# mpotse/ParMmg

Hardware: AMD Instinct MI355X
Metric: new-mesh points located+interpolated/sec (Mpts/s) and HBM GB/s, 1/2/4/8 GPU (higher is better)
Workload: dtype f64

## Files before the change

parmmg_amd/csrc/pmmg_hip.hip:

```cpp
#include <hip/hip_ext.h>
#include <hip/hip_runtime.h>
#ifdef PMMG_HIP_MEASURE
#include <rocprim/device/device_radix_sort.hpp>
#endif

#include <math.h>
#include <stdarg.h>
#include <stdint.h>
#include <stdio.h>
#include <stdlib.h>
#include <string.h>

#include <algorithm>
#include <chrono>
#include <condition_variable>
#include <functional>
#include <mutex>
#include <string>
#include <thread>
#include <type_traits>
#include <vector>

#include "pmmg_device.hpp"
#include "pmmg_prep.hpp"
// ... 93 lines not shown
  st->sorted = sorted;
  st->bin_bits = bits;
}
#endif

}


struct DevBuf {
  void *p = nullptr;
  size_t cap = 0;
};

enum {
  EV_START, EV_FRAME, EV_PREP, EV_ORDER, EV_VOL0, EV_WALK, EV_VOL, EV_JOIN, EV_END, EV_BDY0, EV_BDY1, EV_RESET,
  EV_SB0, EV_ORDER2, EV_SRFSEED, EV_FILL, EV_BDYFB, EV_QUANT, EV_COUNT
};

struct pmmg_hip_ctx {
  int device = 0;
  int options = 0;
  hipStream_t stream = nullptr;
  hipStream_t stream2 = nullptr;
  hipStream_t stream3 = nullptr;
  hipStream_t stream_f = nullptr;
  hipStream_t stream2_hi = nullptr;
  bool srf_prio = false;
  char err[512] = {0};
  Bg bg{};
  int met_size = 0;
  int nfield = 0;
  std::vector<int> fsize;
  std::vector<const double *> fin;
  const double *met = nullptr;
  const double *rec = nullptr;
  int rstride = 0;
  DevBuf o_xyz, o_tetv, o_adja, o_triv, o_adjt, o_met, o_rec;
  std::vector<DevBuf> o_f;
  DevBuf frame, stats, grid, sgrid, order_v, order_b, cont, xq;
  DevBuf cohd;
  DevBuf axh;
  DevBuf bkeys, bkeys2, bvals, bvals2;
  DevBuf rs_hist, rs_csum;
  DevBuf brk_k, brk_k2, brk_v, brk_v2, brk_vinv, brk_tinv, brk_xq, brk_xyz, brk_sol, brk_rec, brk_tmp;
  int brick = 0;
  int set_order = 0;
  int no_fb = 0;
  int stream3_mode = 1;
  int srf_solo = -1;
  void *grid_clean_p = nullptr, *sgrid_clean_p = nullptr;
  long long grid_clean_n = 0, sgrid_clean_n = 0;
  DevBuf qs;
  DevBuf cls_cnt;
  DevBuf oflag;
  DevBuf qmin;
  DevBuf fb_vol, fb_bdy, best, nac, cres, bbest, bnac, bcres;
  DevBuf fbp_vol, fbp_bdy;
  DevBuf fbg_vol_c, fbg_vol_u, fbg_vol_i, fbg_bdy_c, fbg_bdy_u, fbg_bdy_i;
  DevBuf h_xyz, h_cls, h_met, h_elem, h_hit;
  std::vector<DevBuf> h_f;
  hipEvent_t ev[EV_COUNT] = {};
  bool pending = false;
  void *stage[2] = {nullptr, nullptr};
  void *stage_dev[2] = {nullptr, nullptr};
  hipEvent_t stage_ev[2] = {};
  int stage_i = 0;
  struct Pool *pool = nullptr;
  DevBuf o_tet4;
  SnapCache snap_cache;
  hipStream_t cstream = nullptr;
  std::thread snap;
  int snap_ok = 1;
  int verbose = 0;
  int tpc = 8;
  int seed_lanes = 4;
  int seed_v0 = 0;
  int pack_passes = 0;
  int bbox_stride = 64;
  int hist_stride = 256;
  int bdy_bpx = 512;
  int bdy_wave = 0;
  int ev_vol0 = EV_VOL0, ev_vol = EV_VOL;
  int quant_side = 0;
  int fuse_cont = 1;
  int host_order = 1;
  int *flag_host = nullptr;
  int *flag_host_dev = nullptr;
  int bdy_dyn = 0;
  int srf_g = 0;
  int srf_mult = 8;
  int bin_bits = kBinBitsCoherent;
  int bin_qs = 0;
  int maxstep = 1024;
  int fanmax = kFanMax;
  int pad = 0;
  int xcd_run = 64;
  struct Kept {
    DevBuf xyz, met;
    std::vector<DevBuf> f;
    int np = 0, met_size = 0;
    std::vector<int> fsize;
    bool valid = false;
  };
  std::vector<Kept> kept;
  int last_host_np = 0, last_host_met = 0;
  std::vector<int> last_host_fsize;
  int carry_slot = -1, carry_np = 0;
  bool carry_bg = false;
  std::vector<int> carry_src;
  DevBuf carry_dsrc, carry_need, carry_ids, carry_cnt, carry_rows, carry_bc;
  int64_t bytes_up = 0;
  std::vector<pmmg_hip_ctx *> lanes;
  bool borrowed_streams = false;
  ncclComm_t comm = nullptr;
  bool comm_owned = false;
  int comm_rank = 0, comm_size = 0;
  DevBuf ag_send, ag_recv, ag_off, ag_chk;
  int group_lanes = 3;
  struct Pool *lane_pool = nullptr;
  int lane_streams = 1;
  int bdy_first = 0;
  int bdy_after = 0;
  int vol_wait_seed = 0;
  int lane0 = 1;
  int vol_split = 0;
  DevBuf locv, locp;
  static constexpr int kMaxVolChunks = 16;
  int vol_chunks = 4;
  hipStream_t stream_i = nullptr;
  hipEvent_t ev_chunk[2][kMaxVolChunks] = {};
  hipEvent_t ev_interp = nullptr;
  int ixcd_run = -1;
  int null_sync = 0;
  int eager_lanes = 0;
  int wave_time = 0;
  DevBuf wt;
  size_t wt_n = 0;
  int filter_steps = 64;
};

static void set_err(pmmg_hip_ctx *c, const char *fmt, ...) {
  if (!c) return;
  va_list ap;
  va_start(ap, fmt);
  vsnprintf(c->err, sizeof(c->err), fmt, ap);
  va_end(ap);
  fprintf(stderr, "[parmmg_hip] %s\n", c->err);
}

#define HIPCK(ctx, expr)                                                                             \
  do {                                                                                               \
    hipError_t e_ = (expr);                                                                          \
    if (e_ != hipSuccess) {                                                                          \
      set_err((ctx), "%s failed: %s (%s:%d)", #expr, hipGetErrorString(e_), __FILE__, __LINE__);   \
      return 0;                                                                                      \
    }                                                                                                \
  } while (0)

static hipError_t ctx_d2h(pmmg_hip_ctx *c, void *dst, const void *src, size_t n) {
  if (c->null_sync) return hipMemcpy(dst, src, n, hipMemcpyDeviceToHost);
  hipError_t e = hipMemcpyAsync(dst, src, n, hipMemcpyDeviceToHost, c->stream);
  return e != hipSuccess ? e : hipStreamSynchronize(c->stream);
}

static int ensure(pmmg_hip_ctx *c, DevBuf &b, size_t bytes) {
  if (bytes == 0) bytes = 16;
// ... 238 lines not shown
}
constexpr long long kRefillCells = 1LL << 20;

static int env_int(const char *name, int def) {
  const char *e = getenv(name);
  if (e && atoi(e) > 0) return atoi(e);
  return def;
}
static int env_int_any(const char *name, int def) {
  const char *e = getenv(name);
  if (!e || !*e) return def;
  char *end = nullptr;
  const long v = strtol(e, &end, 10);
  return (end && *end == 0) ? (int)v : def;
}

extern "C" {

int pmmg_hip_abi_version(void) { return PMMG_HIP_ABI_VERSION; }
int64_t pmmg_hip_stats_size(void) { return (int64_t)sizeof(pmmg_hip_stats); }

int pmmg_hip_device_count(void) {
  int n = 0;
  if (hipGetDeviceCount(&n) != hipSuccess) return 0;
  return n;
}

static pmmg_hip_ctx *create_ctx(int device, int options, bool srf_prio, pmmg_hip_ctx *share = nullptr) {
  int n = pmmg_hip_device_count();
  if (n <= 0 || device < 0 || device >= n) {
    fprintf(stderr, "[parmmg_hip] no HIP device %d (visible: %d)\n", device, n);
    return nullptr;
  }
  pmmg_hip_ctx *c = new pmmg_hip_ctx();
  c->device = device;
  c->options = options;
#ifdef PMMG_HIP_MEASURE
  if (const char *e = getenv("PMMG_HIP_SRFPRIO"))
    if (*e == '1') c->srf_prio = srf_prio;
#else
  (void)srf_prio;
#endif
  if (share) {
    c->stream = share->stream;
    c->stream2 = share->stream2;
    c->borrowed_streams = true;
  }
  if (hipSetDevice(device) != hipSuccess ||
      (!share && (hipStreamCreateWithFlags(&c->stream, hipStreamNonBlocking) != hipSuccess ||
                  hipStreamCreateWithFlags(&c->stream2, hipStreamNonBlocking) != hipSuccess))) {
    fprintf(stderr, "[parmmg_hip] cannot initialise device %d\n", device);
    delete c;
    return nullptr;
  }
  {
    int evf = 0;
#ifdef PMMG_HIP_MEASURE
    evf = env_int("PMMG_HIP_EVFLAGS", 0);
#endif
    const unsigned fl = evf == 1 ? hipEventDisableSystemFence : (evf == 2 ? hipEventReleaseToDevice : 0u);
    for (int i = 0; i < EV_COUNT; i++)
      (void)hipEventCreateWithFlags(&c->ev[i], (i == EV_FRAME || i == EV_END) ? hipEventDefault : fl);
  }
  c->tpc = std::min(4096, env_int("PMMG_HIP_TPC", c->tpc));
  c->srf_mult = std::min(4096, env_int("PMMG_HIP_SRFMULT", c->srf_mult));
  c->bin_bits = std::min(7, env_int("PMMG_HIP_BINBITS", c->bin_bits));
  c->verbose = env_int("PMMG_HIP_VERBOSE", 0);
  c->maxstep = env_int("PMMG_HIP_MAXSTEP", c->maxstep);
  c->group_lanes = std::min(16, env_int("PMMG_HIP_GROUP_LANES", c->group_lanes));
  c->fanmax = env_int("PMMG_HIP_FANMAX", c->fanmax);
  c->srf_g = std::min(1024, env_int("PMMG_HIP_SRFG", 0));
  c->pack_passes = std::max(0, std::min(2, env_int("PMMG_HIP_PACKPASS", c->pack_passes)));
  if (const char *e = getenv("PMMG_HIP_VOLSPLIT"))
    if (*e == '0' || *e == '1') c->vol_split = *e - '0';
  c->vol_chunks = std::max(1, std::min((int)pmmg_hip_ctx::kMaxVolChunks, env_int("PMMG_HIP_VOLCHUNKS", c->vol_chunks)));
  c->bg.fanmax = c->fanmax;
  c->filter_steps = c->filter_steps < c->maxstep ? c->filter_steps : c->maxstep;
  if (const char *e = getenv("PMMG_HIP_FILTER_STEPS"))
    if (*e && atoi(e) >= 0) c->filter_steps = atoi(e);
#ifdef PMMG_HIP_MEASURE
  c->seed_lanes = std::min(4, env_int("PMMG_HIP_SEEDLANES", c->seed_lanes));
  c->seed_v0 = (env_int("PMMG_HIP_SEEDV0", 0) == 1 ? 1 : 0) | (env_int("PMMG_HIP_SEEDNOATOM", 0) == 1 ? 2 : 0);
  c->bbox_stride = env_int("PMMG_HIP_BBOX", c->bbox_stride);
  c->hist_stride = env_int("PMMG_HIP_HIST", c->hist_stride);
  c->bdy_dyn = (env_int("PMMG_HIP_BDYDYN", 2) == 1 ? 1 : 0) | (env_int("PMMG_HIP_BDYNOINTERP", 0) == 1 ? 2 : 0);
  c->bdy_bpx = env_int("PMMG_HIP_BDYBPX", c->bdy_bpx);
  c->bdy_wave = env_int("PMMG_HIP_BDYWAVE", c->bdy_wave);
  c->host_order = env_int_any("PMMG_HIP_HOSTORDER", c->host_order);
  c->fuse_cont = env_int_any("PMMG_HIP_FUSECONT", c->fuse_cont);
  c->quant_side = env_int("PMMG_HIP_QUANTSIDE", c->quant_side);
  c->bin_qs = env_int("PMMG_HIP_BINQS", 2) == 1;
  c->brick = env_int("PMMG_HIP_BRICK", 0);
  c->srf_solo = env_int_any("PMMG_HIP_SRFSOLO", -1);
  c->set_order = env_int("PMMG_HIP_SETORDER", 0);
  if (const char *e = getenv("PMMG_HIP_XCDRUN"))
    if (*e && atoi(e) >= 0) c->xcd_run = atoi(e);
  c->pad = env_int("PMMG_HIP_PAD", 0);
  c->ixcd_run = env_int_any("PMMG_HIP_IXCDRUN", -1);
  c->null_sync = env_int("PMMG_HIP_NULLSYNC", 0);
  c->eager_lanes = env_int("PMMG_HIP_EAGERLANES", 0);
  c->wave_time = env_int("PMMG_HIP_WAVETIME", 0);
  c->lane_streams = std::max(1, std::min(3, env_int("PMMG_HIP_LANE_STREAMS", c->lane_streams)));
  c->lane0 = env_int_any("PMMG_HIP_LANE0", 1) ? 1 : 0;
  c->bdy_first = env_int("PMMG_HIP_BDYFIRST", 0);
  c->bdy_after = env_int("PMMG_HIP_BDYAFTER", 0);
  c->vol_wait_seed = env_int("PMMG_HIP_VOLWAIT", 0);
  c->no_fb = env_int("PMMG_HIP_NOFB", 0);
  c->stream3_mode = env_int_any("PMMG_HIP_STREAM3", c->stream3_mode);
  if (c->stream3_mode == 2 && hipStreamCreateWithFlags(&c->stream3, hipStreamNonBlocking) != hipSuccess)
    c->stream3 = nullptr;
#endif
  return c;
}

static pmmg_hip_ctx *group_lane(pmmg_hip_ctx *c, int j);

pmmg_hip_ctx *pmmg_hip_create(int device, int options) {
  pmmg_hip_ctx *c = create_ctx(device, options, true);
  if (c && c->eager_lanes)
    for (int j = 0; j < c->group_lanes; j++) (void)group_lane(c, j);
  return c;
}

void pmmg_hip_destroy(pmmg_hip_ctx *c) {
  if (!c) return;
  delete c->lane_pool;
  for (pmmg_hip_ctx *l : c->lanes) pmmg_hip_destroy(l);
  (void)hipSetDevice(c->device);
  (void)snap_join(c);
  (void)hipStreamSynchronize(c->stream);
  (void)hipStreamSynchronize(c->stream2);
  if (c->stream2_hi) (void)hipStreamSynchronize(c->stream2_hi);
  if (c->stream3) (void)hipStreamSynchronize(c->stream3);
  if (c->stream_f) (void)hipStreamSynchronize(c->stream_f);
  if (c->cstream) (void)hipStreamSynchronize(c->cstream);
  if (c->stream_i) {
    (void)hipStreamSynchronize(c->stream_i);
    (void)hipStreamDestroy(c->stream_i);
  }
  for (auto &row : c->ev_chunk)
    for (hipEvent_t &e : row)
      if (e) (void)hipEventDestroy(e);
  if (c->ev_interp) (void)hipEventDestroy(c->ev_interp);
  DevBuf *bufs[] = {&c->o_xyz, &c->o_tetv, &c->o_adja, &c->o_triv, &c->o_adjt, &c->o_met, &c->o_rec, &c->frame,
                    &c->stats, &c->grid, &c->sgrid, &c->order_v, &c->cohd,
                    &c->order_b, &c->cont, &c->xq, &c->qs, &c->axh, &c->bkeys, &c->bkeys2, &c->bvals, &c->bvals2, &c->rs_hist, &c->rs_csum, &c->oflag, &c->cls_cnt, &c->qmin, &c->fb_vol, &c->fb_bdy,
                    &c->best, &c->nac, &c->cres, &c->bbest, &c->bnac, &c->bcres, &c->fbp_vol, &c->fbp_bdy, &c->fbg_vol_c,
                    &c->fbg_vol_u, &c->fbg_vol_i, &c->fbg_bdy_c, &c->fbg_bdy_u, &c->fbg_bdy_i, &c->h_xyz,
                    &c->h_cls, &c->h_met, &c->h_elem, &c->h_hit, &c->brk_k, &c->brk_k2, &c->brk_v, &c->brk_v2,
                    &c->brk_vinv, &c->brk_tinv, &c->brk_xq, &c->brk_xyz, &c->brk_sol, &c->brk_rec, &c->brk_tmp,
                    &c->locv, &c->locp, &c->wt};
  for (DevBuf *b : bufs) release(*b);
  for (auto &b : c->o_f) release(b);
  for (auto &b : c->h_f) release(b);
  for (int i = 0; i < EV_COUNT; i++)
    if (c->ev[i]) (void)hipEventDestroy(c->ev[i]);
  for (int b = 0; b < 2; b++) {
    if (c->stage[b]) (void)hipHostFree(c->stage[b]);
    if (c->stage_ev[b]) (void)hipEventDestroy(c->stage_ev[b]);
  }
  delete c->pool;
  release(c->o_tet4);
  pmmg_snap_cache_free(&c->snap_cache);
  for (auto &k : c->kept) {
    release(k.xyz);
    release(k.met);
// ... 578 lines not shown
    }
    S.s[S.n++] = Slot{c->fin[j], rec_out ? nullptr : fields_out[j], c->fsize[j], c->fsize[j], c->fsize[j]};
  }
  if (c->rec) {
    S.rec = c->rec;
    int off = 0;
    for (int j = 0; j < S.n; j++) {
      S.s[j].in = c->rec + off;
      S.s[j].istride = c->rstride;
      if (rec_out) {
        S.s[j].out = rec_out + off;
        S.s[j].ostride = c->rstride;
      }
      off += S.s[j].code;
    }
    S.rec_out = rec_out;
  }
  const VolPick vpick = pick_layout(S, c->pack_passes);
  if (!vpick.fn) {
    set_err(c, "locate_interp: no packed-record kernel for this slot layout");
    return 0;
  }
  const bool vsplit = S.n > 0 && vpick.ifn && (c->vol_split < 0 ? np_new >= kSmallGroup : c->vol_split == 1);
  LocBuf lb{nullptr, nullptr, nullptr};
  if (vsplit) {
    if (!ensure(c, c->locv, 16 * (size_t)np_new) || !ensure(c, c->locp, 32 * (size_t)np_new)) return 0;
    lb = LocBuf{(nti4 *)c->locv.p, (ntd2 *)c->locp.p, (ntd2 *)c->locp.p + np_new};
    if (!c->stream_i) HIPCK(c, hipStreamCreateWithFlags(&c->stream_i, hipStreamNonBlocking));
    for (auto &row : c->ev_chunk)
      for (hipEvent_t &e : row)
        if (!e) HIPCK(c, hipEventCreateWithFlags(&e, hipEventDisableTiming));
    if (!c->ev_interp) HIPCK(c, hipEventCreateWithFlags(&c->ev_interp, hipEventDisableTiming));
  }
  const VolFn vol_fn = vsplit ? kVolWalk : vpick.fn;
  const int g = grid_dim(bg.ne, c->tpc, 1024);
  const int gs = bg.nt <= 0 ? 1 : (c->srf_g > 0 ? c->srf_g : grid_dim((long long)bg.nt * c->srf_mult, 2, 1024));
  const int gb = 1 << kBinBitsAxis;
  const size_t nq = (size_t)np_new;
  const long long ng = (long long)g * g * g, nsg = bg.nt > 0 ? (long long)gs * gs * gs : 0;
  const long long ncls = (long long)(nq / kScanChunk + 1);
  if (!ensure(c, c->frame, sizeof(Frame)) || !ensure(c, c->stats, sizeof(DevStats) + kStatParts * sizeof(StatPart)) ||
      !ensure(c, c->grid, 8 * (size_t)ng) || !ensure(c, c->sgrid, 8 * (size_t)nsg) || !ensure(c, c->order_v, 4 * nq) ||
      !ensure(c, c->order_b, 4 * nq) || !ensure(c, c->cont, sizeof(ContEntry) * nq) ||
      !ensure(c, c->bkeys, 4 * nq) || !ensure(c, c->bkeys2, 4 * nq) || !ensure(c, c->bvals, 4 * nq) ||
      !ensure(c, c->qs, 24 * nq) || !ensure(c, c->cls_cnt, 4 * (size_t)ncls) || 
      !ensure(c, c->fb_vol, 4 * nq) || !ensure(c, c->fb_bdy, 4 * nq) || !ensure(c, c->best, 4 * nq) ||
      !ensure(c, c->nac, 4 * nq) || !ensure(c, c->cres, 4 * nq) || !ensure(c, c->bbest, 4 * nq) ||
      !ensure(c, c->bnac, 4 * nq) || !ensure(c, c->bcres, 4 * nq) ||
      !ensure(c, c->fbp_vol, sizeof(FbPart) * (size_t)kFbPartCap) ||
      !ensure(c, c->fbp_bdy, sizeof(FbPart) * 256 * (size_t)kFbGridBdy) ||
      !ensure(c, c->fbg_vol_c, 4 * (size_t)(kFbCells + 1)) || !ensure(c, c->fbg_vol_u, 4 * (size_t)kFbCells) ||
      !ensure(c, c->fbg_vol_i, 4 * nq) || !ensure(c, c->fbg_bdy_c, 4 * (size_t)(kFbCells + 1)) ||
      !ensure(c, c->fbg_bdy_u, 4 * (size_t)kFbCells) || !ensure(c, c->fbg_bdy_i, 4 * nq))
    return 0;
  if (!ensure(c, c->xq, sizeof(int) * kXqStride * (size_t)bg.np) || !ensure(c, c->oflag, 2 * sizeof(int)) ||
      !ensure(c, c->cohd, sizeof(double) * kCohSamples) ||
      !ensure(c, c->axh, sizeof(int) * 3 * kMapBins * (size_t)kHistBlocks))
    return 0;
  bg.xq = (const int *)c->xq.p;
  Frame *fr = (Frame *)c->frame.p;
  DevStats *st = (DevStats *)c->stats.p;
  unsigned long long *grid = (unsigned long long *)c->grid.p;
  unsigned long long *sgrid = (unsigned long long *)c->sgrid.p;
  int *order_v = (int *)c->order_v.p, *order_b = (int *)c->order_b.p;
  int force = (c->options & PMMG_HIP_OPT_SORT) ? 1 : (c->options & PMMG_HIP_OPT_NOSORT) ? 0 : -1;
  if (force < 0 && np_new < kSmallGroup) force = 0;
  const bool host_order = force < 0 && c->host_order;
  if (host_order && !c->flag_host) {
    void *p = nullptr;
    HIPCK(c, hipHostMalloc(&p, 64, hipHostMallocCoherent | hipHostMallocMapped));
    c->flag_host = (int *)p;
    void *d = nullptr;
    HIPCK(c, hipHostGetDevicePointer(&d, p, 0));
    c->flag_host_dev = (int *)d;
  }
  if (host_order) c->flag_host[0] = -1;

  const long long ng_clr = (c->grid.p == c->grid_clean_p && ng <= c->grid_clean_n) ? 0 : ng;
  const long long nsg_clr = (c->sgrid.p == c->sgrid_clean_p && nsg <= c->sgrid_clean_n) ? 0 : nsg;
  c->grid_clean_n = c->sgrid_clean_n = 0;
  hipExtLaunchKernelGGL(k_reset, dim3(blocks_for(ng_clr > nsg_clr ? ng_clr : nsg_clr, 2048)), dim3(kBlock), 0, s,
                        c->ev[EV_START], force >= 0 ? c->ev[EV_RESET] : nullptr, 0, fr, st, grid, ng_clr, sgrid,
                        nsg_clr, (int *)c->oflag.p, force, c->bin_bits);
  hipExtLaunchKernelGGL(k_bbox, dim3(std::max(force < 0 ? kCohBlocks : 1, blocks_for(bg.np / c->bbox_stride + 1, 256))),
                        dim3(kBlock), 0, s, nullptr, c->ev[EV_FRAME], 0, (const double *)bg.xyz, bg.np, fr,
                        c->bbox_stride, g, gs, gb, xyz_new, np_new, force < 0 ? (int *)c->oflag.p : nullptr,
                        (double *)c->cohd.p, host_order ? c->flag_host_dev : nullptr);
  const bool quant_side = c->quant_side && np_new >= kSmallGroup;
  if (quant_side) {
    if (!c->stream_f) HIPCK(c, hipStreamCreateWithFlags(&c->stream_f, hipStreamNonBlocking));
    HIPCK(c, hipStreamWaitEvent(c->stream_f, c->ev[EV_FRAME], 0));
    hipLaunchKernelGGL(k_quantize, dim3(blocks_for(3LL * bg.np, 8192)), dim3(kBlock), 0, c->stream_f, bg.xyz,
                       (long long)bg.np, (const Frame *)fr, (int *)c->xq.p, c->hist_stride, (int *)nullptr);
    HIPCK(c, hipEventRecord(c->ev[EV_QUANT], c->stream_f));
    hipLaunchKernelGGL(k_axis_hist, dim3(kHistBlocks), dim3(kBlock), 0, s, bg.xyz, (long long)bg.np,
                       (const Frame *)fr, c->hist_stride, (int *)c->axh.p);
  } else {
    hipLaunchKernelGGL(k_quantize, dim3(std::max(kHistBlocks, blocks_for(3LL * bg.np, 8192))), dim3(kBlock), 0, s,
                       bg.xyz, (long long)bg.np, (const Frame *)fr, (int *)c->xq.p, c->hist_stride, (int *)c->axh.p);
  }
  hipLaunchKernelGGL(k_axis_map, dim3(3), dim3(kBlock), 0, s, (const int *)c->axh.p, fr, g);
  HIPCK(c, hipGetLastError());

  HIPCK(c, hipStreamWaitEvent(sb, c->ev[force < 0 ? EV_FRAME : EV_RESET], 0));
  if (force == 1 || bg.nt <= 0) HIPCK(c, hipEventRecord(c->ev[EV_SB0], sb));
  hipStream_t sc = sb;
  if (force != 0) {
    if (c->stream3_mode == 1 && !c->stream3 &&
        hipStreamCreateWithFlags(&c->stream3, hipStreamNonBlocking) != hipSuccess)
      c->stream3 = nullptr;
    if (c->stream3) sc = c->stream3;
    HIPCK(c, hipStreamWaitEvent(sc, c->ev[EV_FRAME], 0));
  }
  bool split = force < 0 && sc != sb && np_new < (1 << 23);
  HIPCK(c, hipGetLastError());

  {
    const long long nsamp = ng < bg.ne ? ng : bg.ne;
    hipExtLaunchKernelGGL(k_seed_vol, dim3((blocks_for((nsamp + kSeedBatch - 1) / kSeedBatch, 8192) + 7) & ~7),
                          dim3(kBlock), 0, s, nullptr, quant_side ? nullptr : c->ev[EV_PREP], 0, bg, fr, grid, g,
                          nsamp, c->seed_lanes, c->seed_v0, quant_side ? bg.xyz : (const double *)nullptr);
    if (quant_side) {
      HIPCK(c, hipStreamWaitEvent(s, c->ev[EV_QUANT], 0));
      HIPCK(c, hipEventRecord(c->ev[EV_PREP], s));
    }
  }
  HIPCK(c, hipGetLastError());

  const int *flag = (const int *)c->oflag.p;
#ifdef PMMG_HIP_MEASURE
  if (c->set_order) hipLaunchKernelGGL(k_set_order, dim3(1), dim3(1), 0, s, st, force > 0 ? 1 : 0, c->bin_bits);
#endif
  auto launch_cls = [&](bool order_end) -> bool {
    if (force == 1 || bg.nt <= 0) return false;
    int *bc = (int *)c->cls_cnt.p;
    hipExtLaunchKernelGGL(k_cls_count, dim3((unsigned)ncls), dim3(kBlock), 0, sb, c->ev[EV_SB0], nullptr, 0,
                          pclass, (long long)np_new, (int)PMMG_PT_BDY, bc, flag, 0);
    hipLaunchKernelGGL(k_scan_top, dim3(1), dim3(kBlock), 0, sb, bc, (int)ncls, &st->nbdy, flag, 0);
    hipExtLaunchKernelGGL(k_cls_scatter, dim3((unsigned)ncls), dim3(kBlock), 0, sb, nullptr,
                          order_end ? c->ev[EV_ORDER] : nullptr, 0, pclass, (long long)np_new, (int)PMMG_PT_BDY,
                          (const int *)bc, order_b, flag, 0);
    return order_end;
  };
  auto launch_morton = [&]() -> int {
    if (force == 0 || np_new <= 0) return 1;
    const int ntile = (int)((np_new + kRsTile - 1) / kRsTile);
    const long long nh = 256LL * ntile;
    const int nch = (int)((nh + kScanChunk - 1) / kScanChunk);
    if (!ensure(c, c->bvals2, 4 * nq) || !ensure(c, c->rs_hist, 4 * (size_t)nh) || !ensure(c, c->rs_csum, 4 * (size_t)nch))
      return 0;
    unsigned *k0 = (unsigned *)c->bkeys.p, *k1 = (unsigned *)c->bkeys2.p;
    int *v0 = (int *)c->bvals.p, *v1 = (int *)c->bvals2.p, *hist = (int *)c->rs_hist.p, *csum = (int *)c->rs_csum.p;
    const int tgrid = std::min(ntile, kRsGrid);
    hipLaunchKernelGGL(k_bin_keys, dim3(tgrid), dim3(kBlock), 0, sc, xyz_new, pclass, np_new, (const Frame *)fr, flag,
                       k0, v0, st, kRsTile, ntile, hist);
    for (int pass = 0; pass < 3; pass++) {
      const unsigned *kin = pass == 1 ? k1 : k0;
      const int *vin = pass == 1 ? v1 : v0;
      unsigned *kout = pass == 1 ? k0 : k1;
      int *vout = pass == 1 ? v0 : (pass == 0 ? v1 : order_v);
      if (pass > 0)
        hipLaunchKernelGGL(k_rs_hist, dim3(tgrid), dim3(kBlock), 0, sc, kin, np_new, 8 * pass, ntile, hist, flag, 1);
      hipLaunchKernelGGL(k_rs_scan_local, dim3(nch), dim3(kBlock), 0, sc, hist, (int)nh, csum, flag, 1);
      hipLaunchKernelGGL(k_scan_top, dim3(1), dim3(kBlock), 0, sc, csum, nch, (int *)nullptr, flag, 1);
      hipLaunchKernelGGL(k_rs_scan_add, dim3(nch), dim3(kBlock), 0, sc, hist, (int)nh, (const int *)csum, flag, 1);
      hipLaunchKernelGGL(k_rs_scatter, dim3(tgrid), dim3(kBlock), 0, sc, kin, vin, np_new, 8 * pass, ntile,
                         (const int *)hist, kout, vout, flag, 1);
// ... 958 lines not shown
```

parmmg_amd/csrc/pmmg_prep.hpp:

```cpp
#pragma once

#include "pmmg_device.hpp"

namespace pmmg {

struct DevStats {
  int nvol, nbdy;
  int nfb_vol, nfb_bdy;
  int ncont;
  int sorted;
  int bin_bits;
  int pad;
  int bdy_next[8];
  int nac_vol, nac_bdy;
  double fbg_lo[2][3], fbg_inv[2][3];
  int fbg_n[2];
  unsigned walk_done;
  unsigned bdy_done;
  unsigned fb_done[4];
};

struct FbInit {
  int *best;
  __device__ __forceinline__ void at(int slot) const { best[slot] = INT_MAX; }
};

constexpr int kStatParts = 256;
constexpr int kCntVolQueries = 12;
constexpr int kCntWaveIters = 13;
constexpr int kCntExact = 14;
constexpr int kCntNoSeed = 15;
constexpr int kCntStuck = 16;
constexpr int kCntLimit = 17;
constexpr int kCntFanScan = 18;
constexpr int kNumCnt = 20;
struct StatPart {
  unsigned long long cnt[kNumCnt];
  unsigned long long steps;
  unsigned long long stepmax;
};
__device__ __forceinline__ StatPart *stat_part(DevStats *st) {
  return reinterpret_cast<StatPart *>(st + 1) + (blockIdx.x & (kStatParts - 1));
}

struct BlockStats {
  unsigned int cnt[kNumCnt];
  unsigned long long steps;
  unsigned int stepmax;
};

__device__ __forceinline__ void bstats_init(BlockStats *b) {
  if (threadIdx.x < kNumCnt) b->cnt[threadIdx.x] = 0;
  if (threadIdx.x == 0) {
    b->steps = 0;
    b->stepmax = 0;
  }
}

__device__ __forceinline__ void bstats_flush(BlockStats *b, DevStats *st) {
  StatPart *pt = stat_part(st);
  if (threadIdx.x < kNumCnt && b->cnt[threadIdx.x]) atomicAdd(&pt->cnt[threadIdx.x], (unsigned long long)b->cnt[threadIdx.x]);
  if (threadIdx.x == 0) {
    if (b->steps) atomicAdd(&pt->steps, b->steps);
    if (b->stepmax) atomicMax(&pt->stepmax, (unsigned long long)b->stepmax);
  }
}

__device__ __forceinline__ void wave_stats(BlockStats *bs, bool active, int hit, int steps) {
  unsigned int s = active ? (unsigned)steps : 0u, mx = s;
  for (int off = 32; off > 0; off >>= 1) {
    s += __shfl_down(s, off);
    unsigned o = __shfl_down(mx, off);
    mx = o > mx ? o : mx;
  }
  if (__lane_id() == 0) {
    if (s) atomicAdd(&bs->steps, (unsigned long long)s);
    if (mx) {
      atomicMax(&bs->stepmax, mx);
      atomicAdd(&bs->cnt[kCntWaveIters], mx);
    }
  }
  int h = active ? hit : 0;
  unsigned long long any = __ballot(h > 0);
  while (any) {
    int first = __shfl(h, __ffsll((long long)any) - 1);
    unsigned long long same = __ballot(h == first);
    if (__lane_id() == 0) atomicAdd(&bs->cnt[first], (unsigned)__popcll(same));
    any &= ~same;
  }
}

__device__ __forceinline__ void wave_count(BlockStats *bs, int slot, bool pred) {
  const unsigned long long m = __ballot(pred);
  if (__lane_id() == 0 && m) atomicAdd(&bs->cnt[slot], (unsigned)__popcll(m));
}

constexpr int kMapBins = 2048;
constexpr int kMapRatio = 4;
constexpr int kHistBlocks = 32;

constexpr int kSeedAnyParts = 64;
struct Frame {
  unsigned long long key_lo[3], key_hi[3];
  double lo[3], ext[3];
  double inv_vol[3], inv_srf[3], inv_bin[3];
  double qc[3], qs;
  int adaptive;
  int seed_any[kSeedAnyParts];
  unsigned bbox_done;
  float map[3][kMapBins + 1];
};

__device__ __forceinline__ double seed_pos(const Frame *fr, int d, double x, int g) {
  const double u = (x - fr->lo[d]) * fr->inv_vol[d];
  if (!((fr->adaptive >> d) & 1)) return u;
  double b = u * ((double)kMapBins / (double)g);
  b = b > 0.0 ? (b < (double)kMapBins ? b : (double)kMapBins - 1e-9) : 0.0;
  const int i = (int)b;
  const double m0 = fr->map[d][i], m1 = fr->map[d][i + 1];
  return (m0 + (b - (double)i) * (m1 - m0)) * (double)g;
}
__device__ __forceinline__ int seed_cell(double t, int g) {
  const int c = t > 0.0 ? (int)t : 0;
  return c < g ? c : g - 1;
}

constexpr double kQuantHalf = 536870912.0;
__device__ __forceinline__ int quant(double x, const Frame *fr, int d) {
  double t = (x - fr->qc[d]) * fr->qs;
  t = t > 2.0 * kQuantHalf ? 2.0 * kQuantHalf : (t < -2.0 * kQuantHalf ? -2.0 * kQuantHalf : t);
  return __double2int_rn(t);
}

__device__ __forceinline__ void axis_hist_block(int (*h)[kMapBins], const double *xyz, long long np, const Frame *fr,
                                                int stride, int *H) {
  for (int j = threadIdx.x; j < 3 * kMapBins; j += kBlock) (&h[0][0])[j] = 0;
  __syncthreads();
  const long long ns = (np + stride - 1) / stride;
  for (long long j = blockIdx.x * (long long)blockDim.x + threadIdx.x; j < ns; j += (long long)kHistBlocks * blockDim.x) {
    unsigned long long z = (unsigned long long)j * 0x9E3779B97F4A7C15ULL + 0x5EED2025ULL;
    z = (z ^ (z >> 30)) * 0xBF58476D1CE4E5B9ULL;
    z = (z ^ (z >> 27)) * 0x94D049BB133111EBULL;
    z ^= z >> 31;
    const long long i = (long long)(z % (unsigned long long)np);
#pragma unroll
    for (int d = 0; d < 3; d++) {
      const double e = fr->ext[d];
      const double b = e > 0.0 ? (xyz[3 * i + d] - fr->lo[d]) * ((double)kMapBins / e) : 0.0;
      if (b >= 0.0 && b < (double)kMapBins) atomicAdd(&h[d][(int)b], 1);
    }
  }
  __syncthreads();
  for (int j = threadIdx.x; j < 3 * kMapBins; j += kBlock) H[(size_t)blockIdx.x * 3 * kMapBins + j] = (&h[0][0])[j];
}

constexpr int kQuantU = 4;
__global__ __launch_bounds__(kBlock) void k_axis_hist(const double *xyz, long long np, const Frame *fr, int hstride,
                                                      int *H) {
  __shared__ int h[3][kMapBins];
  axis_hist_block(h, xyz, np, fr, hstride, H);
}

__global__ __launch_bounds__(kBlock) void k_quantize(const double *xyz, long long np, const Frame *fr, int *xq,
                                                     int hstride, int *H) {
  __shared__ int h[3][kMapBins];
  if (H && blockIdx.x < kHistBlocks) axis_hist_block(h, xyz, np, fr, hstride, H);
  const long long nth = (long long)gridDim.x * blockDim.x;
  if (kXqStride == 3 && ((uintptr_t)xyz & 15) == 0 && ((uintptr_t)xq & 7) == 0) {
    const double qs = fr->qs, qc0 = fr->qc[0], qc1 = fr->qc[1], qc2 = fr->qc[2];
    const double lim = 2.0 * kQuantHalf;
    auto q = [&](double x, unsigned d) {
      double t = (x - (d == 0 ? qc0 : (d == 1 ? qc1 : qc2))) * qs;
      t = t > lim ? lim : (t < -lim ? -lim : t);
      return __double2int_rn(t);
    };
    const long long n = 3 * np, npair = n / 2;
    const ntd2 *src = reinterpret_cast<const ntd2 *>(xyz);
    nti2 *dst = reinterpret_cast<nti2 *>(xq);
    for (long long p0 = blockIdx.x * (long long)blockDim.x * kQuantU + threadIdx.x; p0 < npair;
         p0 += nth * kQuantU) {
      ntd2 v[kQuantU];
#pragma unroll
      for (int u = 0; u < kQuantU; u++) {
        const long long p = p0 + (long long)u * blockDim.x;
        if (p < npair) v[u] = __builtin_nontemporal_load(src + p);
      }
#pragma unroll
      for (int u = 0; u < kQuantU; u++) {
        const long long p = p0 + (long long)u * blockDim.x;
        if (p < npair) {
          const unsigned d0 = (unsigned)((2 * p) % 3);
          const unsigned d1 = d0 == 2u ? 0u : d0 + 1u;
          const nti2 w = {q(v[u].x, d0), q(v[u].y, d1)};
          __builtin_nontemporal_store(w, dst + p);
        }
      }
    }
    if (blockIdx.x == 0 && threadIdx.x == 0 && (n & 1))
      xq[n - 1] = q(xyz[n - 1], (unsigned)((n - 1) % 3));
    return;
  }
  for (long long j = blockIdx.x * (long long)blockDim.x + threadIdx.x; j < 3 * np; j += nth)
    xq[kXqStride * (j / 3) + j % 3] = quant(__builtin_nontemporal_load(xyz + j), fr, (int)(j % 3));
}

__global__ __launch_bounds__(kBlock) void k_reset(Frame *fr, DevStats *st, unsigned long long *grid, long long ng,
                                                  unsigned long long *sgrid, long long nsg, int *flag, int force,
                                                  int force_bits) {
  const long long tid = blockIdx.x * (long long)blockDim.x + threadIdx.x, nth = (long long)gridDim.x * blockDim.x;
  if (tid < kSeedAnyParts) fr->seed_any[tid] = INT_MAX;
  if (tid == 0) {
    for (int d = 0; d < 3; d++) {
      fr->key_lo[d] = ~0ULL;
      fr->key_hi[d] = 0ULL;
    }
    fr->adaptive = 0;
    fr->bbox_done = 0u;
    if (force >= 0) {
      flag[0] = force;
      flag[1] = force_bits;
    }
    unsigned int *w = reinterpret_cast<unsigned int *>(st);
    for (size_t j = 0; j < sizeof(DevStats) / 4; j++) w[j] = 0u;
  }
  {
    unsigned long long *pw = reinterpret_cast<unsigned long long *>(st + 1);
    for (long long j = tid; j < (long long)(kStatParts * sizeof(StatPart) / 8); j += nth) pw[j] = 0ULL;
  }
  for (long long j = tid; j < ng; j += nth) grid[j] = ~0ULL;
  for (long long j = tid; j < nsg; j += nth) sgrid[j] = ~0ULL;
}

__device__ void frame_final(Frame *fr, int g, int gs, int gb);

constexpr int kCohBlocks = 8, kCohSamples = 4096;
__device__ void coherence_final(const Frame *fr, const double *cohd, int nq, int *flag, int *flag_host);
__device__ __forceinline__ double coh_sample(const double *xyz, int np, int smp) {
  unsigned long long z = (unsigned long long)smp * 0x9E3779B97F4A7C15ULL + 0x5EED2025ULL;
  z = (z ^ (z >> 30)) * 0xBF58476D1CE4E5B9ULL;
  z = (z ^ (z >> 27)) * 0x94D049BB133111EBULL;
  z ^= z >> 31;
  const long long i = (long long)(z % (unsigned long long)(np - 1));
  double d2 = 0.0;
  for (int d = 0; d < 3; d++) {
    const double t = xyz[3 * (size_t)(i + 1) + d] - xyz[3 * (size_t)i + d];
    d2 += t * t;
  }
  return sqrt(d2);
}
__global__ __launch_bounds__(kBlock) void k_bbox(const double *xyz, int np, Frame *fr, int stride, int g, int gs,
                                                 int gb, const double *qxyz, int nq, int *flag, double *cohd,
                                                 int *flag_host) {
  __shared__ unsigned long long slo[3][kBlock / 64], shi[3][kBlock / 64];
  unsigned long long lo[3] = {~0ULL, ~0ULL, ~0ULL}, hi[3] = {0ULL, 0ULL, 0ULL};
  const long long ns = ((long long)np + stride - 1) / stride + 2;
  if (flag && blockIdx.x < kCohBlocks && nq >= 2) {
#pragma unroll
    for (int s = 0; s < kCohSamples / (kCohBlocks * kBlock); s++) {
      const int smp = (blockIdx.x * (kCohSamples / (kCohBlocks * kBlock)) + s) * kBlock + threadIdx.x;
      cohd[smp] = coh_sample(qxyz, nq, smp);
    }
  }
  constexpr int kBboxBatch = 4;
  const long long gs_ = (long long)gridDim.x * blockDim.x;
  for (long long j0 = blockIdx.x * blockDim.x + threadIdx.x; j0 < ns; j0 += kBboxBatch * gs_) {
    double r[kBboxBatch][3];
    bool ok[kBboxBatch];
#pragma unroll
    for (int b = 0; b < kBboxBatch; b++) {
      const long long j = j0 + b * gs_;
      ok[b] = j < ns;
      unsigned long long z = (unsigned long long)j * 0x9E3779B97F4A7C15ULL + 0xB0B0B0B0ULL;
      z = (z ^ (z >> 30)) * 0xBF58476D1CE4E5B9ULL;
      z = (z ^ (z >> 27)) * 0x94D049BB133111EBULL;
      z ^= z >> 31;
      const long long i = !ok[b] || j == 0 ? 0 : (j == 1 ? np - 1 : (long long)(z % (unsigned long long)np));
#pragma unroll
      for (int d = 0; d < 3; d++) r[b][d] = xyz[3 * i + d];
    }
#pragma unroll
    for (int b = 0; b < kBboxBatch; b++)
#pragma unroll
      for (int d = 0; d < 3; d++) {
        const unsigned long long k = dkey(r[b][d]);
        lo[d] = ok[b] && k < lo[d] ? k : lo[d];
        hi[d] = ok[b] && k > hi[d] ? k : hi[d];
      }
  }
#pragma unroll
  for (int d = 0; d < 3; d++) {
    for (int off = 32; off > 0; off >>= 1) {
      unsigned long long a = __shfl_down(lo[d], off), b = __shfl_down(hi[d], off);
      lo[d] = a < lo[d] ? a : lo[d];
      hi[d] = b > hi[d] ? b : hi[d];
    }
  }
  int w = threadIdx.x >> 6, lane = threadIdx.x & 63;
  if (lane == 0)
    for (int d = 0; d < 3; d++) {
      slo[d][w] = lo[d];
      shi[d][w] = hi[d];
    }
  __syncthreads();
  if (threadIdx.x < 3) {
    int d = threadIdx.x;
    unsigned long long a = ~0ULL, b = 0ULL;
    for (int j = 0; j < kBlock / 64; j++) {
      a = slo[d][j] < a ? slo[d][j] : a;
      b = shi[d][j] > b ? shi[d][j] : b;
    }
    atomicMin(&fr->key_lo[d], a);
    atomicMax(&fr->key_hi[d], b);
  }
  __threadfence();
  __syncthreads();
  __shared__ bool last;
  if (threadIdx.x == 0) last = atomicAdd(&fr->bbox_done, 1u) == gridDim.x - 1;
  __syncthreads();
  if (!last) return;
  if (threadIdx.x == 0) {
    __threadfence();
    frame_final(fr, g, gs, gb);
  }
  __syncthreads();
  if (flag) coherence_final(fr, cohd, nq, flag, flag_host);
}

__device__ void frame_final(Frame *fr, int g, int gs, int gb) {
  double emax = 0.0;
  for (int d = 0; d < 3; d++) {
    double lo = dunkey(atomicOr(&fr->key_lo[d], 0ULL)), hi = dunkey(atomicOr(&fr->key_hi[d], 0ULL));
    double ext = hi - lo;
    fr->lo[d] = lo;
    fr->ext[d] = ext;
    fr->inv_vol[d] = ext > 0.0 ? (double)g / ext : 0.0;
    fr->inv_srf[d] = ext > 0.0 ? (double)gs / ext : 0.0;
    fr->inv_bin[d] = ext > 0.0 ? (double)gb / ext : 0.0;
    fr->qc[d] = lo + 0.5 * ext;
    emax = ext > emax ? ext : emax;
  }
  fr->qs = emax > 0.0 ? kQuantHalf / (0.625 * emax) : 1.0;
}

constexpr int kSeedRun = 4;
constexpr unsigned long long kSeedIdMask = (1ULL << 29) - 1;

constexpr int kSeedBatch = 3;
__global__ __launch_bounds__(kBlock) void k_seed_vol(Bg bg, Frame *fr, unsigned long long *cell, int g,
                                                     long long nsamp, int lanes, int v0only, const double *xyzc) {
  constexpr int R = kSeedRun, B = kSeedBatch;
  __shared__ int smin;
  if (threadIdx.x == 0) smin = INT_MAX;
  __syncthreads();
  int kmin = INT_MAX;
  const long long nruns = (nsamp + R - 1) / R;
  const long long quads = bg.ne / 4;
  const long long nthreads = nruns * R;
  const long long per = (nthreads + 8LL * kBlock - 1) / (8LL * kBlock) * kBlock;
  const long long lo = (blockIdx.x & 7) * per, hi = lo + per < nthreads ? lo + per : nthreads;
  const long long bstride = (long long)(gridDim.x >> 3) * blockDim.x;
  const int adaptive = fr->adaptive;
  double sa[3], sb[3];
#pragma unroll
  for (int d = 0; d < 3; d++) {
    sa[d] = (fr->qc[d] - fr->lo[d]) * fr->inv_vol[d];
    sb[d] = 0.25 * fr->inv_vol[d] / fr->qs;
  }
  const int lane = __lane_id(), r = lane % R, g0 = lane - r;
  for (long long s0 = lo + (blockIdx.x >> 3) * (long long)blockDim.x; s0 < hi; s0 += B * bstride) {
    int k[B];
    int4 tv[B];
    bool ok[B];
#pragma unroll
    for (int b = 0; b < B; b++) {
      const long long s = s0 + b * bstride + threadIdx.x;
      const long long run = s / R;
      const long long base = 4 * ((run * quads) / (nruns > 0 ? nruns : 1));
      k[b] = (int)(1 + base + r);
      ok[b] = s < hi && k[b] <= bg.ne && r < lanes;
      tv[b] = make_int4(0, 0, 0, 0);
      if (ok[b]) {
        const nti4 rr =
            __builtin_nontemporal_load(reinterpret_cast<const nti4 *>(bg.tetv + (size_t)(k[b] - 1) * bg.tstride));
        tv[b] = make_int4(rr.x, rr.y, rr.z, rr.w);
      }
    }
    long long sq[B][3];
    double cc[B][3];
#pragma unroll
    for (int b = 0; b < B; b++) {
      ok[b] = ok[b] && tv[b].x > 0;
#pragma unroll
      for (int d = 0; d < 3; d++) {
        cc[b][d] = 0.0;
        sq[b][d] = 0;
      }
      if (xyzc) {
        if (ok[b]) {
          double p0[3], p1[3], p2[3], p3[3];
          load_pt(xyzc, tv[b].x, p0);
          load_pt(xyzc, tv[b].y, p1);
          load_pt(xyzc, tv[b].z, p2);
          load_pt(xyzc, tv[b].w, p3);
#pragma unroll
          for (int d = 0; d < 3; d++) cc[b][d] = 0.25 * ((p0[d] + p1[d]) + (p2[d] + p3[d]));
        }
        continue;
      }
      if (ok[b] && (v0only & 1)) {
        const int *q0 = bg.xq + kXqStride * (size_t)(tv[b].x - 1);
#pragma unroll
        for (int d = 0; d < 3; d++) sq[b][d] = 4LL * q0[d];
      } else if (ok[b]) {
        const int *q0 = bg.xq + kXqStride * (size_t)(tv[b].x - 1), *q1 = bg.xq + kXqStride * (size_t)(tv[b].y - 1);
// ... 240 lines not shown
  int pre = 0, all = 0;
#pragma unroll
  for (int j = 0; j < kBlock / 64; j++) {
    pre += j < w ? wsum[j] : 0;
    all += wsum[j];
  }
  __syncthreads();
  *tot = all;
  return pre + inc - v;
}

__device__ __forceinline__ bool gate_off(const int *gate, int want) { return gate && *gate != want; }

__global__ __launch_bounds__(kBlock) void k_scan_top(int *bsum, int nb, int *total, const int *gate, int want) {
  if (gate_off(gate, want)) return;
  int carry = 0;
  for (int b0 = 0; b0 < nb; b0 += kBlock) {
    const int b = b0 + threadIdx.x;
    const int v = b < nb ? bsum[b] : 0;
    int tot;
    const int pre = block_excl_scan(v, &tot);
    if (b < nb) bsum[b] = carry + pre;
    carry += tot;
  }
  if (threadIdx.x == 0 && total) *total = carry;
}


__global__ __launch_bounds__(kBlock) void k_axis_map(const int *H, Frame *fr, int g) {
  constexpr int R = kMapBins / kBlock;
  const int d = blockIdx.x;
  __shared__ int cum[kMapBins + 1];
  int cnt[R], s = 0;
#pragma unroll
  for (int q = 0; q < R; q++) {
    const int b = R * threadIdx.x + q;
    int v = 0;
#pragma unroll 16
    for (int k = 0; k < kHistBlocks; k++) v += H[(size_t)k * 3 * kMapBins + d * kMapBins + b];
    cnt[q] = v;
    s += v;
  }
  int tot;
  const int pre = block_excl_scan(s, &tot);
  {
    int run = pre;
#pragma unroll
    for (int q = 0; q < R; q++) {
      cum[R * threadIdx.x + q] = run;
      run += cnt[q];
    }
    if (threadIdx.x == kBlock - 1) cum[kMapBins] = run;
  }
  __syncthreads();
  const int W = (kMapBins + g - 1) / (g > 0 ? g : 1);
  int mx = 0;
#pragma unroll
  for (int q = 0; q < R; q++) {
    const int b = R * threadIdx.x + q, e = b + W < kMapBins ? b + W : kMapBins;
    const int w = cum[e] - cum[b];
    mx = w > mx ? w : mx;
  }
  __shared__ int smx[kBlock];
  smx[threadIdx.x] = mx;
  __syncthreads();
  for (int o = kBlock / 2; o > 0; o >>= 1) {
    if (threadIdx.x < o) smx[threadIdx.x] = smx[threadIdx.x + o] > smx[threadIdx.x] ? smx[threadIdx.x + o] : smx[threadIdx.x];
    __syncthreads();
  }
  const bool adapt = tot > 0 && (long long)smx[0] * g > (long long)kMapRatio * tot;
#pragma unroll
  for (int q = 0; q < R; q++) {
    const int b = R * threadIdx.x + q;
    fr->map[d][b] = adapt ? (float)((double)cum[b] / (double)tot) : (float)b / (float)kMapBins;
  }
  if (threadIdx.x == kBlock - 1) fr->map[d][kMapBins] = 1.0f;
  if (threadIdx.x == 0 && adapt) atomicOr(&fr->adaptive, 1 << d);
}


constexpr int kBinBitsAxis = 7;
constexpr int kBinBitsCoherent = 5;

__device__ __noinline__ void coherence_final(const Frame *fr, const double *cohd, int nq, int *flag,
                                             int *flag_host) {
  constexpr int nw = kBlock / 64;
  __shared__ int s_near[nw];
  __threadfence();
  const double vol = fmax(fr->ext[0], 1e-300) * fmax(fr->ext[1], 1e-300) * fmax(fr->ext[2], 1e-300);
  const double h = cbrt(vol / (double)(nq > 1 ? nq : 1));
  int near = 0;
  for (int j = threadIdx.x; nq >= 2 && j < kCohSamples; j += kBlock) near += cohd[j] < 4.0 * h ? 1 : 0;
  for (int o = 32; o > 0; o >>= 1) near += __shfl_xor(near, o);
  if (__lane_id() == 0) s_near[threadIdx.x >> 6] = near;
  __syncthreads();
  if (threadIdx.x == 0) {
    int tot = 0;
    for (int j = 0; j < nw; j++) tot += s_near[j];
    const bool coherent = nq > 1 && 4 * tot >= 3 * kCohSamples;
    flag[0] = coherent ? 0 : 1;
    flag[1] = 2 * tot >= kCohSamples ? kBinBitsCoherent : kBinBitsAxis;
    if (flag_host) {
      flag_host[0] = flag[0];
      flag_host[1] = flag[1];
      __threadfence_system();
    }
  }
}


__global__ __launch_bounds__(kBlock) void k_bin_keys(const double *xyz, const uint8_t *pclass, int np, const Frame *fr,
                                                     const int *flag, unsigned *keys, int *vals, DevStats *st,
                                                     int tile_keys, int ntile, int *hist) {
  if (flag[0] != 1) return;
  const int bits = flag[1];
  __shared__ int h[kBlock];
  __shared__ int sv, sb;
  h[threadIdx.x] = 0;
  if (threadIdx.x == 0) sv = sb = 0;
  __syncthreads();
  int nv = 0, nb = 0;
  for (int tile = blockIdx.x; tile < ntile; tile += gridDim.x) {
  const long long base = (long long)tile * tile_keys;
  constexpr int kBatch = 8;
  for (int e0 = 0; e0 < tile_keys; e0 += kBatch * kBlock) {
    int c[kBatch];
    double x[kBatch][3];
#pragma unroll
    for (int u = 0; u < kBatch; u++) {
      const long long i = base + e0 + u * kBlock + threadIdx.x;
      const bool in = e0 + u * kBlock + (int)threadIdx.x < tile_keys && i < np;
      c[u] = in ? (int)pclass[i] : -1;
#pragma unroll
      for (int d = 0; d < 3; d++) x[u][d] = in ? xyz[3 * i + d] : 0.0;
    }
#pragma unroll
    for (int u = 0; u < kBatch; u++) {
      if (c[u] < 0) continue;
      const long long i = base + e0 + u * kBlock + threadIdx.x;
      unsigned cls = 2u;
      uint32_t q[3] = {0u, 0u, 0u};
      if (c[u] == PMMG_PT_VOL || c[u] == PMMG_PT_BDY) {
        cls = c[u] == PMMG_PT_VOL ? 0u : 1u;
        nv += c[u] == PMMG_PT_VOL;
        nb += c[u] == PMMG_PT_BDY;
#pragma unroll
        for (int d = 0; d < 3; d++)
          q[d] = (uint32_t)cell_coord(x[u][d], fr->lo[d], fr->inv_bin[d], 1 << kBinBitsAxis) >> (kBinBitsAxis - bits);
      }
      const unsigned key = (cls << (3 * bits)) | (expand10(q[0]) << 2) | (expand10(q[1]) << 1) | expand10(q[2]);
      keys[i] = key;
      vals[i] = (int)(i + 1);
      atomicAdd(&h[key & 255u], 1);
    }
  }
  __syncthreads();
  hist[(size_t)threadIdx.x * ntile + tile] = h[threadIdx.x];
  h[threadIdx.x] = 0;
  __syncthreads();
  }
  for (int o = 32; o > 0; o >>= 1) {
    nv += __shfl_down(nv, o);
    nb += __shfl_down(nb, o);
  }
  if (__lane_id() == 0) {
    atomicAdd(&sv, nv);
    atomicAdd(&sb, nb);
  }
  __syncthreads();
  if (threadIdx.x == 0) {
    if (sv) atomicAdd(&st->nvol, sv);
    if (sb) atomicAdd(&st->nbdy, sb);
  }
}

// ... 221 lines not shown
```

Measured before the change: 5549.

## Replace bbox global atomics with per-block partials reduced by last block

```diff
diff --git a/parmmg_amd/csrc/pmmg_hip.hip b/parmmg_amd/csrc/pmmg_hip.hip
--- a/parmmg_amd/csrc/pmmg_hip.hip
+++ b/parmmg_amd/csrc/pmmg_hip.hip
@@ -199,6 +199,7 @@
   int bdy_wave = 0;
   int ev_vol0 = EV_VOL0, ev_vol = EV_VOL;
   int quant_side = 0;
+  int bbox_blocks = kBboxBlocks;
   int fuse_cont = 1;
   int host_order = 1;
   int *flag_host = nullptr;
@@ -603,6 +604,7 @@
   c->seed_lanes = std::min(4, env_int("PMMG_HIP_SEEDLANES", c->seed_lanes));
   c->seed_v0 = (env_int("PMMG_HIP_SEEDV0", 0) == 1 ? 1 : 0) | (env_int("PMMG_HIP_SEEDNOATOM", 0) == 1 ? 2 : 0);
   c->bbox_stride = env_int("PMMG_HIP_BBOX", c->bbox_stride);
+  c->bbox_blocks = std::min(kBboxBlocksMax, env_int("PMMG_HIP_BBOXBLOCKS", c->bbox_blocks));
   c->hist_stride = env_int("PMMG_HIP_HIST", c->hist_stride);
   c->bdy_dyn = (env_int("PMMG_HIP_BDYDYN", 2) == 1 ? 1 : 0) | (env_int("PMMG_HIP_BDYNOINTERP", 0) == 1 ? 2 : 0);
   c->bdy_bpx = env_int("PMMG_HIP_BDYBPX", c->bdy_bpx);
@@ -1347,7 +1349,8 @@
   hipExtLaunchKernelGGL(k_reset, dim3(blocks_for(ng_clr > nsg_clr ? ng_clr : nsg_clr, 2048)), dim3(kBlock), 0, s,
                         c->ev[EV_START], force >= 0 ? c->ev[EV_RESET] : nullptr, 0, fr, st, grid, ng_clr, sgrid,
                         nsg_clr, (int *)c->oflag.p, force, c->bin_bits);
-  hipExtLaunchKernelGGL(k_bbox, dim3(std::max(force < 0 ? kCohBlocks : 1, blocks_for(bg.np / c->bbox_stride + 1, 256))),
+  hipExtLaunchKernelGGL(k_bbox,
+                        dim3(std::max(force < 0 ? kCohBlocks : 1, blocks_for(bg.np / c->bbox_stride + 1, c->bbox_blocks))),
                         dim3(kBlock), 0, s, nullptr, c->ev[EV_FRAME], 0, (const double *)bg.xyz, bg.np, fr,
                         c->bbox_stride, g, gs, gb, xyz_new, np_new, force < 0 ? (int *)c->oflag.p : nullptr,
                         (double *)c->cohd.p, host_order ? c->flag_host_dev : nullptr);
diff --git a/parmmg_amd/csrc/pmmg_prep.hpp b/parmmg_amd/csrc/pmmg_prep.hpp
--- a/parmmg_amd/csrc/pmmg_prep.hpp
+++ b/parmmg_amd/csrc/pmmg_prep.hpp
@@ -100,6 +100,7 @@
 constexpr int kHistBlocks = 32;
 
 constexpr int kSeedAnyParts = 64;
+constexpr int kBboxBlocks = 128, kBboxBlocksMax = 256;
 struct Frame {
   unsigned long long key_lo[3], key_hi[3];
   double lo[3], ext[3];
@@ -109,6 +110,7 @@
   int seed_any[kSeedAnyParts];
   unsigned bbox_done;
   float map[3][kMapBins + 1];
+  alignas(64) unsigned long long bbox_part[kBboxBlocksMax][8];
 };
 
 __device__ __forceinline__ double seed_pos(const Frame *fr, int d, double x, int g) {
@@ -210,10 +212,6 @@
   const long long tid = blockIdx.x * (long long)blockDim.x + threadIdx.x, nth = (long long)gridDim.x * blockDim.x;
   if (tid < kSeedAnyParts) fr->seed_any[tid] = INT_MAX;
   if (tid == 0) {
-    for (int d = 0; d < 3; d++) {
-      fr->key_lo[d] = ~0ULL;
-      fr->key_hi[d] = 0ULL;
-    }
     fr->adaptive = 0;
     fr->bbox_done = 0u;
     if (force >= 0) {
@@ -231,10 +229,12 @@
   for (long long j = tid; j < nsg; j += nth) sgrid[j] = ~0ULL;
 }
 
-__device__ void frame_final(Frame *fr, int g, int gs, int gb);
+__device__ void frame_final(Frame *fr, const unsigned long long *klo, const unsigned long long *khi, int g, int gs, int gb);
 
 constexpr int kCohBlocks = 8, kCohSamples = 4096;
-__device__ void coherence_final(const Frame *fr, const double *cohd, int nq, int *flag, int *flag_host);
+constexpr int kCohPer = kCohSamples / kBlock;
+__device__ __forceinline__ void coherence_decide(const double *ext, const double *cd, int nq, int *flag,
+                                                 int *flag_host);
 __device__ __forceinline__ double coh_sample(const double *xyz, int np, int smp) {
   unsigned long long z = (unsigned long long)smp * 0x9E3779B97F4A7C15ULL + 0x5EED2025ULL;
   z = (z ^ (z >> 30)) * 0xBF58476D1CE4E5B9ULL;
@@ -254,7 +254,8 @@
   __shared__ unsigned long long slo[3][kBlock / 64], shi[3][kBlock / 64];
   unsigned long long lo[3] = {~0ULL, ~0ULL, ~0ULL}, hi[3] = {0ULL, 0ULL, 0ULL};
   const long long ns = ((long long)np + stride - 1) / stride + 2;
-  if (flag && blockIdx.x < kCohBlocks && nq >= 2) {
+  const bool coh = flag && blockIdx.x < kCohBlocks && nq >= 2;
+  if (coh) {
 #pragma unroll
     for (int s = 0; s < kCohSamples / (kCohBlocks * kBlock); s++) {
       const int smp = (blockIdx.x * (kCohSamples / (kCohBlocks * kBlock)) + s) * kBlock + threadIdx.x;
@@ -309,27 +310,75 @@
       a = slo[d][j] < a ? slo[d][j] : a;
       b = shi[d][j] > b ? shi[d][j] : b;
     }
-    atomicMin(&fr->key_lo[d], a);
-    atomicMax(&fr->key_hi[d], b);
-  }
+    unsigned long long *slot = fr->bbox_part[blockIdx.x];
+    __hip_atomic_store(&slot[d], a, __ATOMIC_RELAXED, __HIP_MEMORY_SCOPE_AGENT);
+    __hip_atomic_store(&slot[3 + d], b, __ATOMIC_RELAXED, __HIP_MEMORY_SCOPE_AGENT);
+  }
+  if (coh) __threadfence();
+  __syncthreads();
+  __shared__ bool last;
+  if (threadIdx.x == 0)
+    last = __hip_atomic_fetch_add(&fr->bbox_done, 1u, __ATOMIC_ACQ_REL, __HIP_MEMORY_SCOPE_AGENT) == gridDim.x - 1;
+  __syncthreads();
+  if (!last) return;
   __threadfence();
-  __syncthreads();
-  __shared__ bool last;
-  if (threadIdx.x == 0) last = atomicAdd(&fr->bbox_done, 1u) == gridDim.x - 1;
-  __syncthreads();
-  if (!last) return;
-  if (threadIdx.x == 0) {
-    __threadfence();
-    frame_final(fr, g, gs, gb);
-  }
-  __syncthreads();
-  if (flag) coherence_final(fr, cohd, nq, flag, flag_host);
-}
-
-__device__ void frame_final(Frame *fr, int g, int gs, int gb) {
+#pragma unroll
+  for (int d = 0; d < 3; d++) {
+    lo[d] = ~0ULL;
+    hi[d] = 0ULL;
+  }
+  double cd[kCohPer];
+  const bool test = flag && nq >= 2;
+#pragma unroll
+  for (int u = 0; u < kCohPer; u++) cd[u] = test ? cohd[threadIdx.x + u * kBlock] : 0.0;
+  for (int j = threadIdx.x; j < (int)gridDim.x; j += kBlock) {
+    const unsigned long long *slot = fr->bbox_part[j];
+#pragma unroll
+    for (int d = 0; d < 3; d++) {
+      const unsigned long long a = __hip_atomic_load(&slot[d], __ATOMIC_RELAXED, __HIP_MEMORY_SCOPE_AGENT);
+      const unsigned long long b = __hip_atomic_load(&slot[3 + d], __ATOMIC_RELAXED, __HIP_MEMORY_SCOPE_AGENT);
+      lo[d] = a < lo[d] ? a : lo[d];
+      hi[d] = b > hi[d] ? b : hi[d];
+    }
+  }
+#pragma unroll
+  for (int d = 0; d < 3; d++) {
+    for (int off = 32; off > 0; off >>= 1) {
+      unsigned long long a = __shfl_down(lo[d], off), b = __shfl_down(hi[d], off);
+      lo[d] = a < lo[d] ? a : lo[d];
+      hi[d] = b > hi[d] ? b : hi[d];
+    }
+  }
+  if (lane == 0)
+    for (int d = 0; d < 3; d++) {
+      slo[d][w] = lo[d];
+      shi[d][w] = hi[d];
+    }
+  __syncthreads();
+  unsigned long long klo[3], khi[3];
+  double ext[3];
+#pragma unroll
+  for (int d = 0; d < 3; d++) {
+    klo[d] = ~0ULL;
+    khi[d] = 0ULL;
+#pragma unroll
+    for (int j = 0; j < kBlock / 64; j++) {
+      klo[d] = slo[d][j] < klo[d] ? slo[d][j] : klo[d];
+      khi[d] = shi[d][j] > khi[d] ? shi[d][j] : khi[d];
+    }
+    ext[d] = dunkey(khi[d]) - dunkey(klo[d]);
+  }
+  if (threadIdx.x == 0) frame_final(fr, klo, khi, g, gs, gb);
+  if (flag) coherence_decide(ext, cd, nq, flag, flag_host);
+}
+
+__device__ void frame_final(Frame *fr, const unsigned long long *klo, const unsigned long long *khi, int g, int gs,
+                            int gb) {
   double emax = 0.0;
   for (int d = 0; d < 3; d++) {
-    double lo = dunkey(atomicOr(&fr->key_lo[d], 0ULL)), hi = dunkey(atomicOr(&fr->key_hi[d], 0ULL));
+    fr->key_lo[d] = klo[d];
+    fr->key_hi[d] = khi[d];
+    double lo = dunkey(klo[d]), hi = dunkey(khi[d]);
     double ext = hi - lo;
     fr->lo[d] = lo;
     fr->ext[d] = ext;
@@ -736,15 +785,15 @@
 constexpr int kBinBitsAxis = 7;
 constexpr int kBinBitsCoherent = 5;
 
-__device__ __noinline__ void coherence_final(const Frame *fr, const double *cohd, int nq, int *flag,
-                                             int *flag_host) {
+__device__ __forceinline__ void coherence_decide(const double *ext, const double *cd, int nq, int *flag,
+                                                 int *flag_host) {
   constexpr int nw = kBlock / 64;
   __shared__ int s_near[nw];
-  __threadfence();
-  const double vol = fmax(fr->ext[0], 1e-300) * fmax(fr->ext[1], 1e-300) * fmax(fr->ext[2], 1e-300);
+  const double vol = fmax(ext[0], 1e-300) * fmax(ext[1], 1e-300) * fmax(ext[2], 1e-300);
   const double h = cbrt(vol / (double)(nq > 1 ? nq : 1));
   int near = 0;
-  for (int j = threadIdx.x; nq >= 2 && j < kCohSamples; j += kBlock) near += cohd[j] < 4.0 * h ? 1 : 0;
+#pragma unroll
+  for (int u = 0; u < kCohPer; u++) near += (nq >= 2 && cd[u] < 4.0 * h) ? 1 : 0;
   for (int o = 32; o > 0; o >>= 1) near += __shfl_xor(near, o);
   if (__lane_id() == 0) s_near[threadIdx.x >> 6] = near;
   __syncthreads();
```

Result: no change. 5584, median of 3 (+0.6%).
